# tobiTKM/SPaRC-Gym

Hardware: AMD Instinct MI355X
Metric: env-steps/sec at 65,536 envs, 7x7 grid (HBM roofline fraction in 'roofline') (higher is better)
Workload: dtype u8/u64 (integer bitboards)

## Files before the change

sparc-gym_amd/csrc/sparc_kernels.hip:

```cpp
#include <hip/hip_runtime.h>
#include <dlfcn.h>

#include <algorithm>
#include <atomic>
#include <cstdlib>
#include <cstdio>
#include <cstring>
#include <mutex>
#include <string>
#include <thread>
#include <type_traits>
#include <vector>

#include "sparc_env.hpp"
#include "sparc_trie.hpp"
#include "sparc_movew.hpp"
#include "sparc_move1.hpp"
#include "sparc_rules.hpp"
#include "sparc_snapshot.hpp"
#include "sparc_expand.hpp"
#include "sparc_devbuf.hpp"
#include "sparc_tables.hpp"
#include "sparc_gym_amd.h"

// ... 1040 lines not shown
            }
            if constexpr (!LDS_TABLE) m.tile_end();
            __syncthreads();
        }
        __syncthreads();
        __syncthreads();
        uint4 fs = fin[0], fc;
        if constexpr (IOR) {
            const int32_t* cnt = reinterpret_cast<const int32_t*>(smem + kS_Cnt) + pr * 64u + lane;
            fc = make_uint4((uint32_t)cnt[256], fs.z, 0u, 0u);
            fs.z = (uint32_t)cnt[0];
            fs.w = (uint32_t)cnt[512];
        } else {
            fc = fin[1];
        }
        const uint32_t pend = m.pending ? 1u : 0u;
        m.store(p, i, col, col_addr, fs.x, pend ? (fs.y == 0u ? 1u : 2u) : 0u, fc.y);
        if (stats) {
            const uint32_t resets = p.autoreset == 1 ? pend0 + fc.x - pend : 0u;
            int4 st = stats[i];
            st.x += (int)fs.z;
            st.y += (int)fc.x;
            st.z += (int)fs.w;
            st.w += (int)resets;
            stats[i] = st;
        }
    } else {
        __builtin_amdgcn_s_setprio(1);
        static_assert(!(C && LA), "compact records: the plain trie wave only");
        using TL = TrieLaneT<C>;
        using Rec = typename TL::Rec;
        const Rec* trie = reinterpret_cast<const Rec*>(p.tab.trie8);
        TL tl;
        tl.load(p.st.pos[i], p.st.aux[i], p.st.pid[i], trow, trie, NP);
        const uint32_t* th = reinterpret_cast<const uint32_t*>(pb + kS_FH) + lane;
        uint8_t* tr = pb + kS_Rew + lane;
        static_assert(!(LA && RAND), "the look-ahead trie wave reads the next tile's actions from HBM tiles");
        __syncthreads();
        __syncthreads();
        if constexpr (LA)
            if (K > 0) tl.prime(pb[kS_Act + lane], p.tab.trieg);
        if constexpr (!LDS_TABLE) {
            tl.slot_addr = slot_addr;
            tl.lim = kRowSlots;
        }
        for (int32_t k = 1; k <= K; ++k) {
            const uint8_t* ta = pb + kS_Act + ((k - 1) % 3) * (kTile * 64) + lane;
            if constexpr (!LDS_TABLE) tl.slot_read(kRowSlots, kRowSlotStride);
            const uint32_t a_next = LA ? pb[kS_Act + (k % 3) * (kTile * 64) + lane] : 0u;
#pragma unroll 1
            for (int g = 0; g < kTile; g += kGroup1s) {
                const uint32_t row0 = (uint32_t)((k - 1) * kTile + g) & (kRing - 1);
                uint32_t hb[kGroup1s], av[kGroup1s + 1];
#pragma unroll
                for (int j = 0; j < kGroup1s; ++j) {
                    hb[j] = th[(row0 + j) * 64];
                    av[j] = ta[(g + j) * 64];
                }
                if constexpr (LA) av[kGroup1s] = g + kGroup1s < kTile ? (uint32_t)ta[(g + kGroup1s) * 64] : a_next;
#pragma unroll
                for (int j = 0; j < kGroup1s; ++j) {
                    int code;
                    if constexpr (LA) code = tl.template step1la<!IOR>(hb[j], av[j], av[j + 1], trow, p.tab.trieg, NP);
                    else if constexpr (LDS_TABLE) code = tl.template step1<!IOR>(hb[j], av[j], trow, trie, NP);
                    else code = tl.template step1s<!IOR, kRowSlots, kRowSlotStride>(hb[j], av[j], trow, trie, NP);
                    tr[(row0 + j) * 64] = (uint8_t)code;
                }
            }
            if constexpr (!LDS_TABLE) tl.slot_tile_end(kRowSlots);
            __syncthreads();
        }
        if constexpr (IOR)
            if (K > 0) tl.finish_oneg(th[((uint32_t)(K * kTile - 1) & (kRing - 1)) * 64u] & kHwDone);
        if constexpr (IOR) {
            fin[0] = make_uint4(tl.std_S(), (uint32_t)tl.Oneg, tl.pid, 0u);
        } else {
            fin[0] = make_uint4(tl.std_S(), (uint32_t)tl.Oneg, (uint32_t)tl.acc_x, tl.acc_z);
            fin[1] = make_uint4(tl.acc_y, tl.pid, 0u, 0u);
        }
        __syncthreads();
    }
}

template <int G, int A, int RT>
struct R1Geom {
    static_assert(G * (1 + A) <= 16 && RT % A == 0, "k_rollout1r shape");
    static constexpr int kBlock = 64 * G * (1 + A);
    static constexpr uint32_t kEnvs = 64u * G;
    static constexpr size_t kRing = 0;
    static constexpr size_t kPid = kRing + 2 * RT * kEnvs * 8;
    static constexpr size_t kRew = kPid + 2 * RT * kEnvs * 4;
    static constexpr size_t kFlg = kRew + 3 * RT * kEnvs;
    static constexpr size_t kBits = kFlg + 3 * RT * kEnvs;
    static constexpr size_t kAct = kBits + 2 * RT * kEnvs * 2;
    static constexpr size_t kStk = kAct + G * RT * 64;
    static constexpr size_t kSimple = kStk + (size_t)G * 64 * 64;
    static constexpr size_t kBase = kSimple + 512;
};

template <bool TB, bool RAND, bool LDS_TABLE, int G, int A, int RT, bool INC = false, int WPE = 6>
__global__ void __launch_bounds__(64 * G * (1 + A)) __attribute__((amdgpu_waves_per_eu(WPE)))
    k_rollout1r(Params p, int32_t T, const uint8_t* __restrict__ act, uint64_t seed, uint64_t t0,
                int8_t* __restrict__ rew, uint8_t* __restrict__ flg, int4* __restrict__ stats, uint32_t tiled,
                RulesTab rt, uint16_t* __restrict__ bits) {
    using Geo = R1Geom<G, A, RT>;
    constexpr uint32_t E = Geo::kEnvs;
    extern __shared__ __attribute__((aligned(16))) uint8_t smem[];
    const uint32_t lane = threadIdx.x & 63u, wv = threadIdx.x >> 6;
    const uint32_t g = wv % (uint32_t)G;
    const size_t n = p.n;
    const uint32_t wg_base = blockIdx.x * E;
    const uint32_t col = g * 64u + lane;
    const uint32_t i = wg_base + col;
    const bool active = i < n;
    const bool full = tiled && (size_t)wg_base + E <= n;
    const int32_t K = (T + RT - 1) / RT;
    uint64_t* ring = reinterpret_cast<uint64_t*>(smem + Geo::kRing);
    uint32_t* rpid = reinterpret_cast<uint32_t*>(smem + Geo::kPid);
    uint8_t* trw = smem + Geo::kRew;
    uint8_t* tfl = smem + Geo::kFlg;
    uint16_t* tbt = reinterpret_cast<uint16_t*>(smem + Geo::kBits);
    auto at = [](uint32_t b, int32_t j, uint32_t c) { return (b * (uint32_t)RT + (uint32_t)j) * E + c; };
    auto tile_cnt = [&](int32_t k) { return T - k * RT < RT ? T - k * RT : RT; };
    PuzzleSrc<1> src{p.tab.info, p.tab.root, p.tab.open, p.tab.init, p.tab.row1};
    if constexpr (INC) {
        for (uint32_t k = threadIdx.x; k < 512u; k += Geo::kBlock) smem[Geo::kSimple + k] = (uint8_t)ring_simple(k);
    }
    if constexpr (LDS_TABLE) {
        const uint32_t P = p.tab.num_puzzles;
        uint4* lrow1 = reinterpret_cast<uint4*>(smem + Geo::kBase);
        uint64_t* linit = reinterpret_cast<uint64_t*>(lrow1 + P);
        for (uint32_t k = threadIdx.x; k < P; k += Geo::kBlock) {
            lrow1[k] = p.tab.row1[k];
            linit[k] = p.tab.init[k];
        }
        __syncthreads();
        src = PuzzleSrc<1>{p.tab.info, p.tab.root, p.tab.open, linit, lrow1};
    }

    if (wv < (uint32_t)G) {
        using Stack = typename std::conditional<TB, LdsStack<64>, RegStack>::type;
        Env<1, TB, Stack> e;
        if constexpr (TB) e.stk.col = smem + Geo::kStk + g * 4096u + lane;
        int4 acc = make_int4(0, 0, 0, 0);
        uint64_t initc = 0;
        uint32_t sbit = 0;
        if (active) {
            e.load(p, src, i);
            int c0;
            uint32_t s0;
            e.replay_outputs(c0, s0);
            acc.x -= c0;
            acc.z -= (int)s0;
            initc = src.get_init(e.pid);
            sbit = src.get_row1(e.pid).x & 0xFFu;
        }
        const uint64_t gid = p.env_offset + i;
        uint8_t* ta = smem + Geo::kAct + g * (RT * 64u);
        const uint32_t r = lane >> 2, c = (lane & 3u) * 16u;
        const bool tact = !RAND && full;
        u32x4 anext = {0u, 0u, 0u, 0u};
        if (tact && (int32_t)r < tile_cnt(0)) anext = nt_load16(act + (size_t)r * n + wg_base + g * 64u + c);
        auto store_rf = [&](int32_t kt) {
            const int32_t cnt = tile_cnt(kt);
            const uint32_t b = (uint32_t)kt % 3u;
            if (full) {
                constexpr uint32_t kPer = E / 16u;
                for (uint32_t pi = col; pi < kPer * (uint32_t)cnt; pi += E) {
                    const uint32_t row = pi / kPer, cb = (pi % kPer) * 16u;
                    const size_t o = (size_t)(kt * RT + (int32_t)row) * n + wg_base + cb;
                    if (rew) nt_store16(reinterpret_cast<uint8_t*>(rew) + o, *reinterpret_cast<const u32x4*>(trw + at(b, (int32_t)row, cb)));
                    if (flg) nt_store16(flg + o, *reinterpret_cast<const u32x4*>(tfl + at(b, (int32_t)row, cb)));
                }
            } else if (active) {
                for (int32_t j = 0; j < cnt; ++j) {
                    const size_t o = (size_t)(kt * RT + j) * n + i;
                    if (rew) rew[o] = (int8_t)trw[at(b, j, col)];
                    if (flg) flg[o] = tfl[at(b, j, col)];
                }
            }
        };
        auto store_bits = [&](int32_t kt) {
            const int32_t cnt = tile_cnt(kt);
            const uint32_t b = (uint32_t)kt & 1u;
            if (full) {
                constexpr uint32_t kPer = E / 8u;
                for (uint32_t pi = col; pi < kPer * (uint32_t)cnt; pi += E) {
                    const uint32_t row = pi / kPer, ce = (pi % kPer) * 8u;
                    const size_t o = (size_t)(kt * RT + (int32_t)row) * n + wg_base + ce;
                    nt_store16(reinterpret_cast<uint8_t*>(bits + o), *reinterpret_cast<const u32x4*>(tbt + at(b, (int32_t)row, ce)));
                }
            } else if (active) {
                for (int32_t j = 0; j < cnt; ++j) bits[(size_t)(kt * RT + j) * n + i] = tbt[at(b, j, col)];
            }
        };
        __syncthreads();
        for (int32_t k = 0; k < K; ++k) {
            const int32_t cnt = tile_cnt(k);
            const uint32_t b = (uint32_t)k & 1u;
            if (tact) {
                const u32x4 acur = anext;
                if (k + 1 < K && (int32_t)r < tile_cnt(k + 1))
                    anext = nt_load16(act + (size_t)((k + 1) * RT + (int32_t)r) * n + wg_base + g * 64u + c);
                if ((int32_t)r < cnt) *reinterpret_cast<u32x4*>(ta + r * 64u + c) = acur;
                wave_lds_fence();
            }
#pragma unroll 1
            for (int32_t j = 0; j < cnt; ++j) {
                const int32_t t = k * RT + j;
                uint32_t a = 0;
                if constexpr (RAND) a = uint_rand_action(seed, gid, t0 + (uint64_t)t);
                else if (tact) a = ta[j * 64 + (int32_t)lane];
                else if (active) a = act[(size_t)t * n + i];
                uint32_t f = 0;
                uint64_t w = 0;
                uint32_t q_after = 0;
                if (active) {
                    e.reset_next(p, src);
                    if (e.rs) {
                        initc = e.fr;
                        sbit = e.e;
                    }
                    const int code = e.phase_trie(p);
                    f = e.phase_move(p, a);
                    acc.x += code;
                    acc.z += (int)e.solved;
                    acc.y += (int)e.pending;
                    acc.w += (int)e.s_rs;
                    if (t > 0) {
                        const int32_t tp = t - 1;
                        trw[((uint32_t)(tp / RT) % 3u * (uint32_t)RT + (uint32_t)(tp % RT)) * E + col] = (uint8_t)code;
                    }
                    w = (((initc & ~e.fr) >> p.pitch) | (1ull << sbit)) | ((uint64_t)e.e << kRingShift);
                    q_after = e.pid;
                }
                ring[at(b, j, col)] = w;
                rpid[at(b, j, col)] = q_after;
                tfl[((uint32_t)k % 3u * (uint32_t)RT + (uint32_t)j) * E + col] = (uint8_t)f;
            }
            if (k >= 2) {
                store_rf(k - 2);
                store_bits(k - 2);
            }
            __syncthreads();
        }
        if (active) {
            const int code = e.phase_trie(p);
            acc.x += code;
            acc.z += (int)e.solved;
            const int32_t tp = T - 1;
            trw[((uint32_t)(tp / RT) % 3u * (uint32_t)RT + (uint32_t)(tp % RT)) * E + col] = (uint8_t)code;
        }
        if (K >= 2) {
            store_rf(K - 2);
            store_bits(K - 2);
        }
        __syncthreads();
        store_rf(K - 1);
        store_bits(K - 1);
        if (!active) return;
        e.store(p, src, i);
        if (stats) {
            int4 st = stats[i];
            st.x += acc.x;
            st.y += acc.y;
            st.z += acc.z;
            st.w += acc.w;
            stats[i] = st;
        }
        return;
    }

    __builtin_amdgcn_s_setprio(1);
    const uint32_t q = wv / (uint32_t)G - 1u;
    PuzzleRules<1> pr;
    pr.q = 0xFFFFFFFFu;
    __syncthreads();
    __syncthreads();
    if constexpr (INC) {
        constexpr int32_t BL = RT / A;
        const uint8_t* simple = smem + Geo::kSimple;
        RegionSet1 rs;
        for (int32_t k = 1; k <= K; ++k) {
            const int32_t kt = k - 1, cnt = tile_cnt(kt);
            const uint32_t b = (uint32_t)kt & 1u;
            const int32_t j0 = (int32_t)q * BL, j1 = j0 + BL < cnt ? j0 + BL : cnt;
            if (A > 1) rs.q = 0xFFFFFFFFu;
#pragma unroll 1
            for (int32_t j = j0; j < j1; ++j) {
                const uint64_t w = ring[at(b, j, col)];
                const uint32_t pid = rpid[at(b, j, col)];
                uint32_t out = 0;
                if (active) {
                    if (pr.q != pid) pr = puzzle_rules<1>(p, rt, pid);
                    const uint32_t ab = (uint32_t)(w >> kRingShift) & 63u;
                    out = rs.audit(p, rt, pr, w & ((1ull << kRingShift) - 1ull), ab == pr.tbit, simple);
                }
                tbt[at(b, j, col)] = (uint16_t)out;
            }
            __syncthreads();
        }
        return;
    }
    constexpr uint32_t kSlots = (uint32_t)(A * G) * 64u;
    const uint32_t s0 = (wv - (uint32_t)G) * 64u + lane;
    (void)q;
    for (int32_t k = 1; k <= K; ++k) {
        const int32_t kt = k - 1, cnt = tile_cnt(kt);
        const uint32_t b = (uint32_t)kt & 1u;
#pragma unroll 1
        for (uint32_t J = s0; J < (uint32_t)RT * E; J += kSlots) {
            const uint32_t ec = J / (uint32_t)RT, jj = J - ec * (uint32_t)RT;
            const int32_t j = (int32_t)jj;
            if (j >= cnt) continue;
            const uint64_t w = ring[at(b, j, ec)];
            const uint32_t pid = rpid[at(b, j, ec)];
            uint32_t out = 0;
            if (wg_base + ec < n) {
                if (pid != pr.q) pr = puzzle_rules<1>(p, rt, pid);
                BB<1> vb;
                vb.w[0] = w & ((1ull << kRingShift) - 1ull);
                const uint32_t ab = (uint32_t)(w >> kRingShift) & 63u;
                out = audit_r<1, NoMemo, true>(p, rt, pr, vb, ab == pr.tbit, nullptr, nullptr).bits;
            }
            tbt[at(b, j, ec)] = (uint16_t)out;
        }
        __syncthreads();
    }
}

constexpr size_t kW_Act = 0, kW_Rew = 2 * kTile * 64, kW_Hand = kW_Rew + kRing * 64, kW_Board = kW_Hand + 2 * kRing * 64;
__host__ __device__ constexpr size_t splitw_fin_bytes() { return 4 * 64 * 2 * sizeof(uint4); }

template <int W, bool TB, bool RAND, bool LDS_TABLE, bool IOR = false>
__global__ void __launch_bounds__(kBlock1s) k_rolloutWs(Params p, SplitGeom g, const uint4* __restrict__ mrow,
                                                        const uint32_t* __restrict__ boards, int32_t T,
                                                        const uint8_t* __restrict__ act, uint64_t seed, uint64_t t0,
                                                        int8_t* __restrict__ rew, uint8_t* __restrict__ flg,
                                                        int4* __restrict__ stats) {
    extern __shared__ __attribute__((aligned(16))) uint8_t smem[];
    const uint32_t lane = threadIdx.x & 63u, wv = threadIdx.x >> 6;
    const uint32_t NP = p.tab.num_puzzles;
    const size_t fin_off = 4 * (size_t)g.pair;
    const uint4* trow = p.tab.trow;
    if constexpr (LDS_TABLE) {
        uint4* lt = reinterpret_cast<uint4*>(smem + fin_off + splitw_fin_bytes());
        for (uint32_t k = threadIdx.x; k < NP; k += kBlock1s) lt[k] = p.tab.trow[k];
        __syncthreads();
        trow = lt;
    }
    const size_t n = p.n;
    const uint32_t wg_base = blockIdx.x * 256u;
    const int32_t K = T / kTile;

    int32_t* const cnt = reinterpret_cast<int32_t*>(smem + fin_off + 256 * sizeof(uint4));
    if (wv >= 8) {
        const uint32_t io = wv - 8u;
        const uint32_t r = lane >> 2, c = (lane & 3u) * 16u;
        IoCounters ct;
        auto load_tile = [&](int32_t k) {
            if constexpr (!RAND) {
// ... 325 lines not shown
    int dev = -1;
    DevGuard() {
        if (hipGetDevice(&dev) != hipSuccess) dev = -1;
    }
    ~DevGuard() {
        int cur = -1;
        if (dev >= 0 && hipGetDevice(&cur) == hipSuccess && cur != dev) (void)hipSetDevice(dev);
    }
    DevGuard(const DevGuard&) = delete;
    DevGuard& operator=(const DevGuard&) = delete;
};

Params make_params(const Ctx* c, const PuzzleDev& z) {
    Params p{};
    p.tab.open = z.open.get();
    p.tab.info = z.info.get();
    p.tab.root = z.root.get();
    p.tab.trie = z.trie.get();
    p.tab.init = z.init.get();
    p.tab.row1 = z.row1.get();
    p.tab.trie8 = z.trie8.get();
    p.tab.trieg = z.trieg.get();
    p.tab.trow = z.trow.get();
    p.tab.mrow = z.mrow.get();
    p.tab.num_puzzles = z.num_puzzles;
    p.st.vis = c->vis.get();
    p.st.dirs = c->dirs.get();
    p.st.pos = c->pos.get();
    p.st.aux = c->aux.get();
    p.st.step = c->step.get();
    p.st.pid = c->pid.get();
    p.n = c->n;
    p.pitch = (uint32_t)c->cfg.pitch;
    p.max_steps = c->cfg.max_steps;
    p.autoreset = c->cfg.autoreset;
    p.env_offset = (uint64_t)c->cfg.env_offset;
    p.err = c->err.get();
    const uint32_t P = p.pitch;
    p.nbr_pos = (2u * P) | ((P - 1u) << 8) | (0u << 16) | ((P + 1u) << 24);
    if (c->W == 1 && split1_pitch_ok(P)) {
        p.nbm = window_nbm(P);
        p.lmagic = legal_magic(P);
    }
    return p;
}
Params make_params(const Ctx* c) { return make_params(c, c->pz); }

inline dim3 grid_for(size_t n) { return dim3((unsigned)((n + kBlock - 1) / kBlock)); }

int allow_big_lds(Ctx* c, const void* kern) {
    static std::mutex mu;
    static std::vector<std::pair<int, const void*>> done;
    std::lock_guard<std::mutex> lock(mu);
    for (const auto& k : done)
        if (k.first == c->device && k.second == kern) return SPARC_OK;
    HIPCHK(c, hipFuncSetAttribute(kern, hipFuncAttributeMaxDynamicSharedMemorySize, (int)kMaxDynLds));
    done.emplace_back(c->device, kern);
    return SPARC_OK;
}

template <class F>
void dispatch_w_tb(int w, bool tb, F&& f) {
    using T1 = std::integral_constant<int, 1>;
    using T2 = std::integral_constant<int, 2>;
    using T4 = std::integral_constant<int, 4>;
    if (w == 1) tb ? f(T1{}, std::true_type{}) : f(T1{}, std::false_type{});
    else if (w == 2) tb ? f(T2{}, std::true_type{}) : f(T2{}, std::false_type{});
    else tb ? f(T4{}, std::true_type{}) : f(T4{}, std::false_type{});
}

int check_ctx(Ctx* c, bool need_state) {
    if (!c) return fail(nullptr, SPARC_E_INVALID, "null context");
    if (!c->loaded) return fail(c, SPARC_E_STATE, "sparc_load_puzzles has not been called");
    if (need_state && !c->has_state) return fail(c, SPARC_E_STATE, "sparc_reset has not been called");
    HIPCHK(c, hipSetDevice(c->device));
    return SPARC_OK;
}

int launch_check(Ctx* c) {
    HIPCHK(c, hipGetLastError());
    return SPARC_OK;
}

template <int G_, int A_, int RT_, bool INC_ = false, int WPE_ = 6>
struct R1Shape {
    static constexpr int G = G_, A = A_, RT = RT_, WPE = WPE_;
    static constexpr bool INC = INC_;
};

constexpr uint64_t kFitQueueCap = 1u << 16;
constexpr uint64_t kFitQueueMax = (uint64_t)1 << 28;

RulesTab rules_tab(const Ctx* c, const RuleDev& r, bool queue) {
    RulesTab rt{};
    rt.planes = r.planes.get();
    rt.inst_fc = r.inst_fc.get();
    rt.inst = r.inst.get();
    rt.shape_range = r.shape_range.get();
    rt.shape_area = r.shape_area.get();
    rt.shape_off = r.shape_off.get();
    rt.num_puzzles = c->pz.num_puzzles;
    rt.area = r.area ? 1u : 0u;
    rt.fit_cap = c->fit_cap;
    rt.reg_off = r.reg_off.get();
    rt.reg_tab = r.reg_tab.get();
    rt.fq = FitQueue{queue ? c->fq_count.get() : nullptr, c->fq_items.get(), c->fq_items.size()};
    rt.hf = c->hostfits_off ? HostFits{nullptr, 0u, 0u}
                            : HostFits{c->d_hf.get(), c->h_hf.empty() ? 0u : (uint32_t)c->h_hf.size() - 1u, c->d_hf ? c->hf_used : 0u};
    rt.rows = r.rows.get();
    return rt;
}

template <int W>
int host_fit_w(const Ctx* c, const RuleDev& r, uint32_t q, uint64_t rm) {
    const uint32_t w0 = c->pz.h_info[q].x, X = w0 & 0xFFu, Y = (w0 >> 8) & 0xFFu;
    RulesTab rt{};
    rt.inst = r.h_inst.data();
    rt.shape_range = r.h_shape_range.data();
    rt.shape_off = r.h_shape_off.data();
    const uint2 fc = r.h_inst_fc[q];
    const FitIn fin = fit_in(rt, fc.x, fc.y & ~kHostFit, X, Y);
    const uint32_t P = (uint32_t)c->cfg.pitch;
    BB<W> Rc = BB<W>::zero();
    for (uint32_t b = 0; b < fin.CX * fin.CY; ++b)
        if ((rm >> b) & 1ull) Rc.set((2 * (b / fin.CY) + 1) * P + 2 * (b % fin.CY) + 1);
    if (fc.y & kHostFit) return exact_fit<W, uint64_t, kHostFitMax, kHostFitMax, kHostFitPlanes>(fin, Rc, rm, ~0ull);
    return exact_fit<W, uint64_t>(fin, Rc, rm, ~0ull);
}
int host_fit(const Ctx* c, const RuleDev& r, uint32_t q, uint64_t rm) {
    return c->W == 1 ? host_fit_w<1>(c, r, q, rm) : c->W == 2 ? host_fit_w<2>(c, r, q, rm) : host_fit_w<4>(c, r, q, rm);
}

template <class F>
void parallel_for(size_t n, F&& fn) {
    std::atomic<size_t> next{0};
    auto work = [&]() {
        for (size_t k; (k = next.fetch_add(1)) < n;) fn(k);
    };
    const size_t nt = std::min<size_t>({n, 16, (size_t)std::max(1u, std::thread::hardware_concurrency())});
    std::vector<std::thread> pool;
    for (size_t k = 1; k < nt; ++k) pool.emplace_back(work);
    work();
    for (auto& th : pool) th.join();
}

}

extern "C" {

int sparc_abi_version(void) { return SPARC_ABI_VERSION; }

const char* sparc_last_error(const void* ctx) {
    return ctx ? static_cast<const Ctx*>(ctx)->msg.c_str() : g_err.c_str();
}

int sparc_create(int device, const sparc_config* cfg, void** ctx_out) {
    DevGuard dg;
    if (!cfg || !ctx_out) return fail(nullptr, SPARC_E_INVALID, "null argument");
    *ctx_out = nullptr;
    if (cfg->num_envs < 1) return fail(nullptr, SPARC_E_INVALID, "num_envs must be >= 1");
    if (cfg->words != 1 && cfg->words != 2 && cfg->words != 4)
        return fail(nullptr, SPARC_E_INVALID, "words must be 1, 2 or 4");
    if (cfg->pitch < 1 || cfg->pitch > 255) return fail(nullptr, SPARC_E_INVALID, "pitch must be in 1..255");
    if (cfg->traceback != 0 && cfg->traceback != 1) return fail(nullptr, SPARC_E_INVALID, "traceback must be 0/1");
    if (cfg->autoreset != SPARC_AUTORESET_NONE && cfg->autoreset != SPARC_AUTORESET_NEXT_STEP)
        return fail(nullptr, SPARC_E_INVALID, "unknown autoreset mode");
    int ndev = 0;
    if (hipGetDeviceCount(&ndev) != hipSuccess || ndev == 0)
        return fail(nullptr, SPARC_E_HIP, "no HIP device available");
    if (device < 0 || device >= ndev) return fail(nullptr, SPARC_E_INVALID, "bad device ordinal");
    Ctx* c = new Ctx();
// ... 222 lines not shown
                           (!rtr || aligned(rtr->bits));
    const bool half = false;
    if (c->W == 1 && !ot && !rtr) {
        const size_t blocks = (c->n + 255) / 256;
        const size_t per_cu = (blocks + 255) / 256;
        const size_t budget = std::min(kMaxDynLds, (size_t)160 * 1024 / (per_cu ? per_cu : 1));
        const size_t tbytes = table_lds_bytes<1>(c->pz.num_puzzles);
        if (tiled && c->n % 256 == 0 && T >= kTile && c->pz.trie8 && split1_pitch_ok((uint32_t)c->cfg.pitch)) {
            const int32_t T16 = T / kTile * kTile;
            const size_t sbytes = split_table_bytes(c->pz.num_puzzles);
            const bool lds_s = kS_Base + sbytes <= budget;
            const size_t shm_s = kS_Base + (lds_s ? sbytes : kS_SlotBytes);
            const bool compact = !lds_s && c->pz.trie4 && (c->mixed_trie == 1 || (c->mixed_trie == 0 && c->pz.mixed_pays));
            Params ps = p;
            if (compact) {
                ps.tab.trie8 = reinterpret_cast<const uint2*>(c->pz.trie4.get());
                ps.tab.trow = c->pz.trow4.get();
            }
            auto launch_s = [&](auto kern, const uint8_t* a) {
                if (shm_s > 64 * 1024 && (lds_rc = allow_big_lds(c, reinterpret_cast<const void*>(kern)))) return;
                kern<<<dim3((unsigned)blocks), kBlock1s, shm_s, c->stream>>>(ps, T16, a, seed, t0, d_rew, d_flags, st);
            };
            auto launch_s1 = [&](auto kern, const uint8_t* a) {
                if (shm_s > 64 * 1024 && (lds_rc = allow_big_lds(c, reinterpret_cast<const void*>(kern)))) return;
                kern<<<dim3((unsigned)(4 * blocks)), kBlock1s / 4, shm_s, c->stream>>>(ps, T16, a, seed, t0, d_rew, d_flags,
                                                                                     st);
            };
            auto go_s = [&](auto tb, auto ior) {
                constexpr bool TB = decltype(tb)::value, IOR = decltype(ior)::value;
                if (d_act) {
                    if (lds_s && blocks <= 64) launch_s1(k_rollout1s<TB, false, true, true, IOR, false, 1>, d_act);
                    else if (lds_s) launch_s(k_rollout1s<TB, false, true, false, IOR>, d_act);
                    else if (compact) launch_s(k_rollout1s<TB, false, false, false, IOR, true>, d_act);
                    else launch_s(k_rollout1s<TB, false, false, false, IOR>, d_act);
                } else {
                    if (lds_s) launch_s(k_rollout1s<TB, true, true, false, IOR>, nullptr);
                    else if (compact) launch_s(k_rollout1s<TB, true, false, false, IOR, true>, nullptr);
                    else launch_s(k_rollout1s<TB, true, false, false, IOR>, nullptr);
                }
            };
            const bool ior = p.autoreset == 1 && !c->io_codes_off;
            if (c->cfg.traceback) {
                if (ior) go_s(std::true_type{}, std::true_type{});
                else go_s(std::true_type{}, std::false_type{});
            } else {
                if (ior) go_s(std::false_type{}, std::true_type{});
                else go_s(std::false_type{}, std::false_type{});
            }
            if (lds_rc) return lds_rc;
            rc = launch_check(c);
            if (rc || T16 == T) return rc;
            const size_t adv = (size_t)T16 * c->n;
            if (d_act) d_act += adv;
            if (d_rew) d_rew += adv;
            if (d_flags) d_flags += adv;
            t0 += (uint64_t)T16;
            T -= T16;
        }
        const bool lds_table = kW1Base + tbytes <= budget;
        const size_t shm = kW1Base + (lds_table ? tbytes : 0);
        auto launch = [&](auto kern, const uint8_t* a) {
            if (shm > 64 * 1024 && (lds_rc = allow_big_lds(c, reinterpret_cast<const void*>(kern)))) return;
            kern<<<dim3((unsigned)blocks), kBlock1, shm, c->stream>>>(p, T, a, seed, t0, d_rew, d_flags, st, tiled);
        };
        auto go1 = [&](auto tb) {
            constexpr bool TB = decltype(tb)::value;
            if (d_act) {
                if (lds_table) launch(k_rollout1<TB, false, true>, d_act);
                else launch(k_rollout1<TB, false, false>, d_act);
            } else {
                if (lds_table) launch(k_rollout1<TB, true, true>, nullptr);
                else launch(k_rollout1<TB, true, false>, nullptr);
            }
        };
        if (c->cfg.traceback) go1(std::true_type{});
        else go1(std::false_type{});
        if (lds_rc) return lds_rc;
        return launch_check(c);
    }
    if (rtr && r1r_rollout(c)) {
        auto go_shape = [&](auto geo_c) {
            using Geo = decltype(geo_c);
            constexpr int G = Geo::G, A = Geo::A, RT = Geo::RT, WPE = Geo::WPE;
            constexpr bool INC = Geo::INC;
            using GG = R1Geom<G, A, RT>;
            const size_t blocks = (c->n + GG::kEnvs - 1) / GG::kEnvs;
            const size_t tbytes = table_lds_bytes<1>(c->pz.num_puzzles);
            const bool lds_table = GG::kBase + tbytes <= (GG::kBlock <= 768 ? (size_t)80 * 1024 : kMaxDynLds);
            const size_t shm = GG::kBase + (lds_table ? tbytes : 0);
            auto launch = [&](auto kern, const uint8_t* a) {
                if (shm > 64 * 1024 && (lds_rc = allow_big_lds(c, reinterpret_cast<const void*>(kern)))) return;
                kern<<<dim3((unsigned)blocks), GG::kBlock, shm, c->stream>>>(p, T, a, seed, t0, d_rew, d_flags, st, tiled,
                                                                            rtr->rt, rtr->bits);
            };
            auto go = [&](auto tb) {
                constexpr bool TB = decltype(tb)::value;
                if (d_act) {
                    if (lds_table) launch(k_rollout1r<TB, false, true, G, A, RT, INC, WPE>, d_act);
                    else launch(k_rollout1r<TB, false, false, G, A, RT, INC, WPE>, d_act);
                } else {
                    if (lds_table) launch(k_rollout1r<TB, true, true, G, A, RT, INC, WPE>, nullptr);
                    else launch(k_rollout1r<TB, true, false, G, A, RT, INC, WPE>, nullptr);
                }
            };
            if (c->cfg.traceback) go(std::true_type{});
            else go(std::false_type{});
        };
        switch (c->r1r_shape) {
            case 1: go_shape(R1Shape<4, 3, 12>{}); break;
            case 2: go_shape(R1Shape<2, 4, 12>{}); break;
            case 3: go_shape(R1Shape<4, 1, 4, true, 4>{}); break;
            case 4: go_shape(R1Shape<2, 3, 15, true, 4>{}); break;
            case 5: go_shape(R1Shape<2, 5, 10>{}); break;
            default: go_shape(R1Shape<2, 5, 15>{}); break;
        }
        if (lds_rc) return lds_rc;
        return launch_check(c);
    }
    if (c->W > 1 && !ot && !rtr && c->pz.split_w && tiled && c->n % 256 == 0 && T >= kTile) {
        const int32_t T16 = T / kTile * kTile;
        const SplitGeom& g = c->pz.sgeom;
        const size_t blocks = c->n / 256;
        const size_t base = 4 * (size_t)g.pair + splitw_fin_bytes();
        const bool lds_t = base + sizeof(uint4) * c->pz.num_puzzles <= kMaxDynLds;
        const size_t shm = base + (lds_t ? sizeof(uint4) * c->pz.num_puzzles : 0);
        dispatch_w_tb(c->W, c->cfg.traceback, [&](auto w, auto tb) {
            constexpr int W = decltype(w)::value;
            constexpr bool TB = decltype(tb)::value;
            if constexpr (W > 1) {
                auto launch = [&](auto kern, const uint8_t* a) {
                    if (shm > 64 * 1024 && (lds_rc = allow_big_lds(c, reinterpret_cast<const void*>(kern)))) return;
                    kern<<<dim3((unsigned)blocks), kBlock1s, shm, c->stream>>>(p, g, c->pz.mroww.get(), c->pz.boardw.get(), T16, a, seed,
                                                                              t0, d_rew, d_flags, st);
                };
                auto go = [&](auto ior) {
                    constexpr bool IOR = decltype(ior)::value;
                    if (d_act) {
                        if (lds_t) launch(k_rolloutWs<W, TB, false, true, IOR>, d_act);
                        else launch(k_rolloutWs<W, TB, false, false, IOR>, d_act);
                    } else {
                        if (lds_t) launch(k_rolloutWs<W, TB, true, true, IOR>, nullptr);
                        else launch(k_rolloutWs<W, TB, true, false, IOR>, nullptr);
                    }
                };
                if (p.autoreset == 1 && !c->io_codes_off) go(std::true_type{});
                else go(std::false_type{});
            }
        });
        if (lds_rc) return lds_rc;
        rc = launch_check(c);
        if (rc || T16 == T) return rc;
        const size_t adv = (size_t)T16 * c->n;
        if (d_act) d_act += adv;
        if (d_rew) d_rew += adv;
        if (d_flags) d_flags += adv;
        t0 += (uint64_t)T16;
        T -= T16;
    }
    if (ot && !c->obs_inline) {
        dispatch_w_tb(c->W, c->cfg.traceback, [&](auto w, auto tb) {
            constexpr int W = decltype(w)::value;
            constexpr bool TB = decltype(tb)::value;
            const size_t shm = obsw_lds_bytes<W, TB>();
            const dim3 g((unsigned)((c->n + 255) / 256));
            auto launch = [&](auto kern, const uint8_t* a) {
                if (shm > 64 * 1024 && (lds_rc = allow_big_lds(c, reinterpret_cast<const void*>(kern)))) return;
                kern<<<g, kBlockOw, shm, c->stream>>>(p, T, a, seed, t0, d_rew, d_flags, st, *ot);
            };
            if (d_act) launch(k_rollout_obsw<W, TB, false>, d_act);
            else launch(k_rollout_obsw<W, TB, true>, nullptr);
        });
        if (lds_rc) return lds_rc;
        return launch_check(c);
    }
    dispatch_w_tb(c->W, c->cfg.traceback, [&](auto w, auto tb) {
        constexpr int W = decltype(w)::value;
        constexpr bool TB = decltype(tb)::value;
        auto go = [&](auto epw_c, auto obs_c, auto rules_c) {
            constexpr int EPW = decltype(epw_c)::value;
            constexpr bool OBS = decltype(obs_c)::value;
            constexpr bool RULES = decltype(rules_c)::value;
            if constexpr (W == 1 && !OBS && !RULES) return;
            constexpr size_t kEnvsPerBlock = (size_t)kWaves * EPW / (RULES ? kAuditWaves : 1);
            const size_t blocks = (c->n + kEnvsPerBlock - 1) / kEnvsPerBlock;
            const size_t per_cu = (blocks + 255) / 256;
            const size_t budget = std::min(kMaxDynLds, (size_t)160 * 1024 / (per_cu ? per_cu : 1));
            const size_t base = tiles_lds_bytes<W, EPW>() + stack_lds_bytes<W, TB, EPW>() + (OBS ? obs_lds_bytes<W>() : 0) +
                                (RULES ? bits_lds_bytes<EPW>() : 0);
            const size_t tbytes = table_lds_bytes<W>(c->pz.num_puzzles);
            const bool lds_table = base + tbytes <= budget;
            const size_t shm = base + (lds_table ? tbytes : 0);
            const dim3 g((unsigned)blocks);
            auto launch = [&](auto kern, const uint8_t* a) {
                if (shm > 64 * 1024 && (lds_rc = allow_big_lds(c, reinterpret_cast<const void*>(kern)))) return;
                kern<<<g, kBlock, shm, c->stream>>>(p, T, a, seed, t0, d_rew, d_flags, st, tiled, ot ? *ot : no_obs,
                                                    rtr ? *rtr : no_rules);
            };
// ... 295 lines not shown
        if (cnt > c->fq_items.size()) return fail(c, SPARC_E_STATE, "exact-fit queue overflow on the re-run");
    }
    std::vector<FitTodo> todo(cnt);
    HIPCHK(c, hipMemcpy(todo.data(), c->fq_items.get(), sizeof(FitTodo) * cnt, hipMemcpyDeviceToHost));
    c->fq_last = cnt;
    for (const FitTodo& it : todo)
        if (it.pos >= a.extent || it.q >= c->pz.num_puzzles)
            return fail(c, SPARC_E_STATE, "exact-fit queue entry outside the last audit call");
    std::vector<std::pair<uint32_t, uint64_t>> keys(cnt);
    for (uint64_t k = 0; k < cnt; ++k) keys[k] = {todo[k].q, todo[k].rm};
    std::sort(keys.begin(), keys.end());
    keys.erase(std::unique(keys.begin(), keys.end()), keys.end());
    std::vector<int8_t> res(keys.size(), 0);
    parallel_for(keys.size(), [&](size_t k) { res[k] = (int8_t)host_fit(c, c->rl, keys[k].first, keys[k].second); });
    auto fits = [&](uint32_t q, uint64_t rm) {
        const auto it = std::lower_bound(keys.begin(), keys.end(), std::make_pair(q, rm));
        return res[(size_t)(it - keys.begin())] == 1;
    };
    std::sort(todo.begin(), todo.end(), [](const FitTodo& x, const FitTodo& y) { return x.pos < y.pos; });
    std::vector<RulePatch> patch;
    for (size_t k = 0; k < todo.size();) {
        RulePatch r{todo[k].pos, 0ull, SPARC_RULE_SEARCH_EXHAUSTED, 0u};
        bool ok = true;
        for (; k < todo.size() && todo[k].pos == r.pos; ++k) {
            const bool f = fits(todo[k].q, todo[k].rm);
            ok &= f;
            if (f) r.fit_or |= 1ull << (todo[k].rid & 63u);
        }
        if (!ok) r.clear |= SPARC_RULE_POLY_YLOP | SPARC_RULE_ALL;
        patch.push_back(r);
    }
    DevBuf<RulePatch> d_patch;
    HIPCHK(c, upload(d_patch, patch, c->stream));
    k_rule_patch<<<grid_for(patch.size()), kBlock, 0, c->stream>>>(d_patch.get(), (uint32_t)patch.size(), d_bits, d_fit);
    rc = launch_check(c);
    HIPCHK(c, hipMemsetAsync(c->fq_count.get(), 0, sizeof(unsigned long long), c->stream));
    if (!rc) rc = hostfits_add(c, keys, res);
    HIPCHK(c, hipStreamSynchronize(c->stream));
    return rc;
}
}

extern "C" {

int sparc_rules_device(void* ctx, uint16_t* d_bits, uint8_t* d_region, uint64_t* d_fit) {
    DevGuard dg;
    Ctx* c = static_cast<Ctx*>(ctx);
    int rc = check_ctx(c, true);
    if (rc) return rc;
    if (!c->rules) return fail(c, SPARC_E_STATE, "sparc_load_rules has not been called");
    HIPCHK(c, hipMemsetAsync(c->fq_count.get(), 0, sizeof(unsigned long long), c->stream));
    AuditCall a;
    a.kind = 1;
    a.extent = c->n;
    a.bits = d_bits;
    a.region = d_region;
    a.fit = d_fit;
    c->last_audit = a;
    return launch_rules(c, a);
}

int sparc_rules_queue_stats(void* ctx, uint64_t* out) {
    Ctx* c = static_cast<Ctx*>(ctx);
    if (!c || !out) return fail(c, SPARC_E_INVALID, "null argument");
    out[0] = c->fq_items.size();
    out[1] = c->fq_last;
    out[2] = c->fq_reruns;
    return SPARC_OK;
}

int sparc_set_variant(void* ctx, int32_t which, int32_t value) {
    Ctx* c = static_cast<Ctx*>(ctx);
    if (!c) return fail(nullptr, SPARC_E_INVALID, "null context");
    switch (which) {
        case SPARC_VARIANT_IO_CODES_OFF:
            if (value != 0 && value != 1) break;
            c->io_codes_off = value == 1;
            return SPARC_OK;
        case SPARC_VARIANT_RULE_ROLLOUT_GENERIC:
            if (value != 0 && value != 1) break;
            c->rules_generic = value == 1;
            return SPARC_OK;
        case SPARC_VARIANT_R1R_SHAPE:
            if (value < 0 || value > 5) break;
            c->r1r_shape = value;
            return SPARC_OK;
        case SPARC_VARIANT_OBS_INLINE:
            if (value != 0 && value != 1) break;
            c->obs_inline = value == 1;
            return SPARC_OK;
        case SPARC_VARIANT_MIXED_TRIE:
            if (value < 0 || value > 2) break;
            c->mixed_trie = value;
            return SPARC_OK;
        case SPARC_VARIANT_HOST_FITS:
            if (value != 0 && value != 1) break;
            c->hostfits_off = value == 1;
            return SPARC_OK;
        default:
            return fail(c, SPARC_E_INVALID, "unknown variant");
    }
    return fail(c, SPARC_E_INVALID, "bad variant value");
}

int sparc_set_rule_limits(void* ctx, uint32_t fit_cap_nodes, uint64_t table_entries) {
    DevGuard dg;
    Ctx* c = static_cast<Ctx*>(ctx);
    if (!c) return fail(nullptr, SPARC_E_INVALID, "null context");
    c->fit_cap = fit_cap_nodes ? fit_cap_nodes : kFitCap;
    c->reg_entries = table_entries ? (size_t)std::min<uint64_t>(table_entries, (uint64_t)1 << 28) : (size_t)1 << 28;
    return SPARC_OK;
}

int sparc_rules_finish(void* ctx, uint16_t* d_bits, uint64_t* d_fit) {
    DevGuard dg;
    Ctx* c = static_cast<Ctx*>(ctx);
    int rc = check_ctx(c, false);
    if (rc) return rc;
    if (!c->rules) return fail(c, SPARC_E_STATE, "sparc_load_rules has not been called");
    uint64_t cnt = 0;
    if ((rc = read_queue_count(c, cnt))) return rc;
    return finish_queue(c, cnt, d_bits, d_fit);
}

int sparc_rules_host(void* ctx, uint16_t* bits, uint8_t* region, uint64_t* fit) {
    DevGuard dg;
    Ctx* c = static_cast<Ctx*>(ctx);
    int rc = check_ctx(c, true);
    if (rc) return rc;
    const size_t n = c->n, rb = n * 64 * c->W;
    if ((rc = audit_scratch(c))) return rc;
    rc = sparc_rules_device(c, c->s_bits.get(), region ? c->s_region.get() : nullptr, fit ? c->s_fit.get() : nullptr);
    if (rc) return rc;
    HIPCHK(c, c->h_count.ensure(hipHostMallocDefault));
    HIPCHK(c, hipMemcpyAsync(c->h_count.get(), c->fq_count.get(), sizeof(uint64_t), hipMemcpyDeviceToHost, c->stream));
    if (bits) HIPCHK(c, hipMemcpyAsync(bits, c->s_bits.get(), 2 * n, hipMemcpyDeviceToHost, c->stream));
    if (region) HIPCHK(c, hipMemcpyAsync(region, c->s_region.get(), rb, hipMemcpyDeviceToHost, c->stream));
    if (fit) HIPCHK(c, hipMemcpyAsync(fit, c->s_fit.get(), 8 * n, hipMemcpyDeviceToHost, c->stream));
    HIPCHK(c, hipStreamSynchronize(c->stream));
    const uint64_t cnt = *c->h_count.get();
    if ((rc = finish_queue(c, cnt, c->s_bits.get(), fit ? c->s_fit.get() : nullptr)) || cnt == 0) return rc;
    if (bits) HIPCHK(c, hipMemcpyAsync(bits, c->s_bits.get(), 2 * n, hipMemcpyDeviceToHost, c->stream));
    if (fit) HIPCHK(c, hipMemcpyAsync(fit, c->s_fit.get(), 8 * n, hipMemcpyDeviceToHost, c->stream));
    return sparc_sync(c);
}

}

namespace {
int env_call(Ctx* c, int32_t env, int32_t op, uint32_t arg, int32_t audit, sparc_env_record* out) {
    int rc = check_ctx(c, op != 2);
    if (rc) return rc;
    if (!out) return fail(c, SPARC_E_INVALID, "null record");
    if (env < 0 || (uint32_t)env >= c->n) return fail(c, SPARC_E_INVALID, "env index out of range");
    if (op == 2 && !c->has_state && c->n != 1)
        return fail(c, SPARC_E_STATE, "first reset must cover every env (sparc_reset_*)");
    if (op == 2 && arg >= c->pz.num_puzzles) return fail(c, SPARC_E_INVALID, "puzzle index out of range");
    if (audit && !c->rules) return fail(c, SPARC_E_STATE, "sparc_load_rules has not been called");
    HIPCHK(c, c->h_rec.ensure(hipHostMallocMapped));
    const Params p = make_params(c);
    dispatch_w_tb(c->W, c->cfg.traceback, [&](auto w, auto tb) {
        k_env_op<decltype(w)::value, decltype(tb)::value><<<1, 64, 0, c->stream>>>(p, (uint32_t)env, op, arg, c->h_rec.dev());
    });
    if ((rc = launch_check(c))) return rc;
    if (op == 2) c->has_state = true;
    if (audit) {
        if ((rc = audit_scratch(c))) return rc;
// ... 477 lines not shown
```

sparc-gym_amd/csrc/sparc_layout.hpp:

```cpp
#pragma once
#include <stddef.h>
#include <stdint.h>

#if defined(__HIP__)
#define SPARC_HD __attribute__((host)) __attribute__((device))
#else
#define SPARC_HD
#endif

namespace sparc {

constexpr uint32_t kNone = 0xFFFFu;
constexpr size_t kMaxDynLds = 160 * 1024;

SPARC_HD constexpr bool split1_pitch_ok(uint32_t P) { return P >= 3u && P <= 9u; }

struct SplitGeom {
    uint32_t P2;
    uint32_t B;
    uint32_t BS;
    uint32_t M;
    uint32_t nbr_pos;
    uint32_t pair;
    uint32_t off_board, off_stack;
};
constexpr uint32_t kBoardRegs = 4;

constexpr uint32_t kRingShift = 57;

constexpr size_t kMixedTrieBytes = (size_t)4 << 20;
constexpr uint32_t kHotWalk = 8;

enum : uint32_t {
    RP_CELLS = 0, RP_LATTICE, RP_GAPS, RP_DOTS, RP_TRI, RP_TRI0, RP_TRI1, RP_TRI2, RP_STAR, RP_SQUARE,
    RP_COLORED, RP_COL1, RP_M0 = RP_COL1 + 8, RP_M1, RP_M2, RP_NOTFIRST, RP_NOTLAST, RP_INST, RP_ABI,
    RP_AREA0 = RP_ABI, RP_COUNT = RP_AREA0 + 8
};
constexpr int kAreaPlanes = 8;
constexpr int kFitYlops = 16;
constexpr int kFitShapes = 16;
constexpr int kHostFitMax = 64, kHostFitPlanes = 8;
constexpr uint32_t kHostFit = 0x80000000u;

SPARC_HD inline __attribute__((always_inline)) uint32_t hostfit_slot(uint32_t q, uint64_t rm, uint32_t mask) {
    uint64_t h = rm * 0x9E3779B97F4A7C15ull ^ ((uint64_t)q * 0xC2B2AE3D27D4EB4Full);
    h ^= h >> 29;
    return (uint32_t)h & mask;
}

template <int W>
SPARC_HD constexpr uint32_t rule_row_u64() { return 10u * W + 2u; }
constexpr uint32_t kBasePlanes[10] = {RP_CELLS, RP_LATTICE, RP_GAPS, RP_DOTS, RP_TRI, RP_TRI0, RP_TRI1, RP_TRI2,
                                      RP_NOTFIRST, RP_NOTLAST};
constexpr uint32_t kNoRegTab = 0xFFFFFFFFu;
constexpr uint32_t kRegTabCells = 12;

}
```

Before: 411.5 billion.

## Deduplicate identical audit jobs per tile and compact them into an LDS job list

Adds a DISTINCT variant of the rollout kernel where audit waves first find, for each env within a tile, the steps whose ring word and puzzle id match an earlier step. Only the first occurrence of each is kept, and those are compacted via ballot, atomicAdd and mbcnt into a shared-memory job list. Audit waves then balance work across the compacted list and copy each result to the duplicate steps. Extra __syncthreads are added so producer waves hand off mid-tile. This becomes the new default shape and costs extra LDS, barriers and equality-scan work.

```diff
diff --git a/sparc-gym_amd/csrc/sparc_kernels.hip b/sparc-gym_amd/csrc/sparc_kernels.hip
--- a/sparc-gym_amd/csrc/sparc_kernels.hip
+++ b/sparc-gym_amd/csrc/sparc_kernels.hip
@@ -1146,9 +1146,9 @@
     }
 }
 
-template <int G, int A, int RT>
+template <int G, int A, int RT, bool DISTINCT = false>
 struct R1Geom {
-    static_assert(G * (1 + A) <= 16 && RT % A == 0, "k_rollout1r shape");
+    static_assert(G * (1 + A) <= 16 && (RT % A == 0 || DISTINCT), "k_rollout1r shape");
     static constexpr int kBlock = 64 * G * (1 + A);
     static constexpr uint32_t kEnvs = 64u * G;
     static constexpr size_t kRing = 0;
@@ -1159,15 +1159,20 @@
     static constexpr size_t kAct = kBits + 2 * RT * kEnvs * 2;
     static constexpr size_t kStk = kAct + G * RT * 64;
     static constexpr size_t kSimple = kStk + (size_t)G * 64 * 64;
-    static constexpr size_t kBase = kSimple + 512;
+    static constexpr size_t kList = kSimple + 512;
+    static constexpr size_t kBase = kList + (DISTINCT ? 2 * RT * kEnvs + 16 : 0);
+    static_assert(!DISTINCT || (RT <= 16 && kEnvs <= 4096u), "a job is ec << 4 | j in 16 bits");
 };
 
-template <bool TB, bool RAND, bool LDS_TABLE, int G, int A, int RT, bool INC = false, int WPE = 6>
+template <bool TB, bool RAND, bool LDS_TABLE, int G, int A, int RT, bool INC = false, int WPE = 6, bool DISTINCT = false>
 __global__ void __launch_bounds__(64 * G * (1 + A)) __attribute__((amdgpu_waves_per_eu(WPE)))
     k_rollout1r(Params p, int32_t T, const uint8_t* __restrict__ act, uint64_t seed, uint64_t t0,
                 int8_t* __restrict__ rew, uint8_t* __restrict__ flg, int4* __restrict__ stats, uint32_t tiled,
                 RulesTab rt, uint16_t* __restrict__ bits) {
-    using Geo = R1Geom<G, A, RT>;
+    static_assert(!(INC && DISTINCT), "k_rollout1r: INC keeps regions from step to step, DISTINCT skips steps");
+    constexpr int32_t kMarkSteps = 4;
+    (void)kMarkSteps;
+    using Geo = R1Geom<G, A, RT, DISTINCT>;
     constexpr uint32_t E = Geo::kEnvs;
     extern __shared__ __attribute__((aligned(16))) uint8_t smem[];
     const uint32_t lane = threadIdx.x & 63u, wv = threadIdx.x >> 6;
@@ -1190,6 +1195,13 @@
     if constexpr (INC) {
         for (uint32_t k = threadIdx.x; k < 512u; k += Geo::kBlock) smem[Geo::kSimple + k] = (uint8_t)ring_simple(k);
     }
+    uint16_t* jlist = reinterpret_cast<uint16_t*>(smem + Geo::kList);
+    uint32_t* jcnt = reinterpret_cast<uint32_t*>(smem + Geo::kList + 2 * RT * E);
+    if constexpr (DISTINCT) {
+        if (threadIdx.x < 2u) jcnt[threadIdx.x] = 0u;
+    }
+    (void)jlist;
+    (void)jcnt;
     if constexpr (LDS_TABLE) {
         const uint32_t P = p.tab.num_puzzles;
         uint4* lrow1 = reinterpret_cast<uint4*>(smem + Geo::kBase);
@@ -1204,6 +1216,7 @@
 
     if (wv < (uint32_t)G) {
         using Stack = typename std::conditional<TB, LdsStack<64>, RegStack>::type;
+        if constexpr (DISTINCT) __builtin_amdgcn_s_setprio(1);
         Env<1, TB, Stack> e;
         if constexpr (TB) e.stk.col = smem + Geo::kStk + g * 4096u + lane;
         int4 acc = make_int4(0, 0, 0, 0);
@@ -1271,6 +1284,9 @@
             }
 #pragma unroll 1
             for (int32_t j = 0; j < cnt; ++j) {
+                if constexpr (DISTINCT) {
+                    if (j == kMarkSteps) __syncthreads();
+                }
                 const int32_t t = k * RT + j;
                 uint32_t a = 0;
                 if constexpr (RAND) a = uint_rand_action(seed, gid, t0 + (uint64_t)t);
@@ -1302,6 +1318,9 @@
                 rpid[at(b, j, col)] = q_after;
                 tfl[((uint32_t)k % 3u * (uint32_t)RT + (uint32_t)j) * E + col] = (uint8_t)f;
             }
+            if constexpr (DISTINCT) {
+                if (cnt <= kMarkSteps) __syncthreads();
+            }
             if (k >= 2) {
                 store_rf(k - 2);
                 store_bits(k - 2);
@@ -1315,6 +1334,7 @@
             const int32_t tp = T - 1;
             trw[((uint32_t)(tp / RT) % 3u * (uint32_t)RT + (uint32_t)(tp % RT)) * E + col] = (uint8_t)code;
         }
+        if constexpr (DISTINCT) __syncthreads();
         if (K >= 2) {
             store_rf(K - 2);
             store_bits(K - 2);
@@ -1335,12 +1355,73 @@
         return;
     }
 
-    __builtin_amdgcn_s_setprio(1);
+    if constexpr (!DISTINCT) __builtin_amdgcn_s_setprio(1);
     const uint32_t q = wv / (uint32_t)G - 1u;
     PuzzleRules<1> pr;
     pr.q = 0xFFFFFFFFu;
     __syncthreads();
+    if constexpr (DISTINCT) __syncthreads();
     __syncthreads();
+    if constexpr (DISTINCT) {
+        constexpr uint32_t kSlots = (uint32_t)(A * G) * 64u;
+        constexpr uint32_t kJobs = (uint32_t)RT * E;
+        constexpr uint32_t kRounds = (kJobs + kSlots - 1u) / kSlots;
+        const uint32_t aw = wv - (uint32_t)G;
+        const uint32_t s0 = aw * 64u + lane;
+        for (int32_t k = 1; k <= K; ++k) {
+            const int32_t kt = k - 1, cnt = tile_cnt(kt);
+            const uint32_t b = (uint32_t)kt & 1u;
+            const uint64_t* rw = ring + at(b, 0, 0);
+            const uint32_t* rq = rpid + at(b, 0, 0);
+            uint32_t* const cw = jcnt + ((uint32_t)k & 1u);
+            uint64_t own[kRounds];
+            uint32_t total = 0;
+#pragma unroll
+            for (uint32_t r = 0; r < kRounds; ++r) {
+                const uint32_t J = (aw * kRounds + r) * 64u + lane;
+                const uint32_t ec = J / (uint32_t)RT, j = J - ec * (uint32_t)RT;
+                bool mine = false;
+                if (J < kJobs && (int32_t)j < cnt) {
+                    if (wg_base + ec < n) mine = tile_rep(tile_equal_mask<RT>(rw + ec, rq + ec, E, j), j) == j;
+                    else tbt[at(b, (int32_t)j, ec)] = 0;
+                }
+                own[r] = __ballot(mine);
+                total += (uint32_t)__popcll(own[r]);
+            }
+            uint32_t base = 0;
+            if (lane == 0u && total) base = atomicAdd(cw, total);
+            base = (uint32_t)__builtin_amdgcn_readfirstlane((int)base);
+#pragma unroll
+            for (uint32_t r = 0; r < kRounds; ++r) {
+                const uint32_t J = (aw * kRounds + r) * 64u + lane;
+                const uint32_t ec = J / (uint32_t)RT, j = J - ec * (uint32_t)RT;
+                const uint32_t rank = __builtin_amdgcn_mbcnt_hi((uint32_t)(own[r] >> 32),
+                                                                __builtin_amdgcn_mbcnt_lo((uint32_t)own[r], 0u));
+                if (((own[r] >> lane) & 1ull) && base + rank < kJobs) jlist[base + rank] = (uint16_t)(ec << 4 | j);
+                base += (uint32_t)__popcll(own[r]);
+            }
+            __syncthreads();
+            const uint32_t listed = *cw < kJobs ? *cw : kJobs;
+            if (threadIdx.x == (uint32_t)G * 64u) jcnt[((uint32_t)k + 1u) & 1u] = 0u;
+#pragma unroll 1
+            for (uint32_t s = s0; s < listed; s += kSlots) {
+                const uint32_t e = jlist[s];
+                const uint32_t ec = e >> 4, j = e & 15u;
+                const uint64_t w = rw[j * E + ec];
+                const uint32_t pid = rq[j * E + ec];
+                if (pid != pr.q) pr = puzzle_rules<1>(p, rt, pid);
+                BB<1> vb;
+                vb.w[0] = w & ((1ull << kRingShift) - 1ull);
+                const uint32_t ab = (uint32_t)(w >> kRingShift) & 63u;
+                const uint32_t out = audit_r<1, NoMemo, true>(p, rt, pr, vb, ab == pr.tbit, nullptr, nullptr).bits;
+                tbt[at(b, (int32_t)j, ec)] = (uint16_t)out;
+                for (uint32_t f = tile_followers(tile_equal_mask<RT>(rw + ec, rq + ec, E, j), j, (uint32_t)cnt); f; f &= f - 1u)
+                    tbt[at(b, __builtin_ctz(f), ec)] = (uint16_t)out;
+            }
+            __syncthreads();
+        }
+        return;
+    }
     if constexpr (INC) {
         constexpr int32_t BL = RT / A;
         const uint8_t* simple = smem + Geo::kSimple;
@@ -1832,11 +1913,12 @@
     return SPARC_OK;
 }
 
-template <int G_, int A_, int RT_, bool INC_ = false, int WPE_ = 6>
+template <int G_, int A_, int RT_, bool INC_ = false, int WPE_ = 6, bool DISTINCT_ = false>
 struct R1Shape {
     static constexpr int G = G_, A = A_, RT = RT_, WPE = WPE_;
-    static constexpr bool INC = INC_;
+    static constexpr bool INC = INC_, DISTINCT = DISTINCT_;
 };
+constexpr int kR1rDefault = 9;
 
 constexpr uint64_t kFitQueueCap = 1u << 16;
 constexpr uint64_t kFitQueueMax = (uint64_t)1 << 28;
@@ -2225,8 +2307,8 @@
         auto go_shape = [&](auto geo_c) {
             using Geo = decltype(geo_c);
             constexpr int G = Geo::G, A = Geo::A, RT = Geo::RT, WPE = Geo::WPE;
-            constexpr bool INC = Geo::INC;
-            using GG = R1Geom<G, A, RT>;
+            constexpr bool INC = Geo::INC, DISTINCT = Geo::DISTINCT;
+            using GG = R1Geom<G, A, RT, DISTINCT>;
             const size_t blocks = (c->n + GG::kEnvs - 1) / GG::kEnvs;
             const size_t tbytes = table_lds_bytes<1>(c->pz.num_puzzles);
             const bool lds_table = GG::kBase + tbytes <= (GG::kBlock <= 768 ? (size_t)80 * 1024 : kMaxDynLds);
@@ -2239,23 +2321,26 @@
             auto go = [&](auto tb) {
                 constexpr bool TB = decltype(tb)::value;
                 if (d_act) {
-                    if (lds_table) launch(k_rollout1r<TB, false, true, G, A, RT, INC, WPE>, d_act);
-                    else launch(k_rollout1r<TB, false, false, G, A, RT, INC, WPE>, d_act);
+                    if (lds_table) launch(k_rollout1r<TB, false, true, G, A, RT, INC, WPE, DISTINCT>, d_act);
+                    else launch(k_rollout1r<TB, false, false, G, A, RT, INC, WPE, DISTINCT>, d_act);
                 } else {
-                    if (lds_table) launch(k_rollout1r<TB, true, true, G, A, RT, INC, WPE>, nullptr);
-                    else launch(k_rollout1r<TB, true, false, G, A, RT, INC, WPE>, nullptr);
+                    if (lds_table) launch(k_rollout1r<TB, true, true, G, A, RT, INC, WPE, DISTINCT>, nullptr);
+                    else launch(k_rollout1r<TB, true, false, G, A, RT, INC, WPE, DISTINCT>, nullptr);
                 }
             };
             if (c->cfg.traceback) go(std::true_type{});
             else go(std::false_type{});
         };
-        switch (c->r1r_shape) {
+        switch (c->r1r_shape ? c->r1r_shape : kR1rDefault) {
             case 1: go_shape(R1Shape<4, 3, 12>{}); break;
             case 2: go_shape(R1Shape<2, 4, 12>{}); break;
             case 3: go_shape(R1Shape<4, 1, 4, true, 4>{}); break;
             case 4: go_shape(R1Shape<2, 3, 15, true, 4>{}); break;
             case 5: go_shape(R1Shape<2, 5, 10>{}); break;
-            default: go_shape(R1Shape<2, 5, 15>{}); break;
+            case 6: go_shape(R1Shape<2, 5, 15>{}); break;
+            case 7: go_shape(R1Shape<2, 5, 13, false, 6, true>{}); break;
+            case 8: go_shape(R1Shape<2, 5, 14, false, 6, true>{}); break;
+            case 9: go_shape(R1Shape<2, 5, 15, false, 6, true>{}); break;
         }
         if (lds_rc) return lds_rc;
         return launch_check(c);
@@ -2717,7 +2802,7 @@
             c->rules_generic = value == 1;
             return SPARC_OK;
         case SPARC_VARIANT_R1R_SHAPE:
-            if (value < 0 || value > 5) break;
+            if (value < 0 || value > 9) break;
             c->r1r_shape = value;
             return SPARC_OK;
         case SPARC_VARIANT_OBS_INLINE:
diff --git a/sparc-gym_amd/csrc/sparc_layout.hpp b/sparc-gym_amd/csrc/sparc_layout.hpp
--- a/sparc-gym_amd/csrc/sparc_layout.hpp
+++ b/sparc-gym_amd/csrc/sparc_layout.hpp
@@ -28,6 +28,26 @@
 
 constexpr uint32_t kRingShift = 57;
 
+template <int RT>
+SPARC_HD inline __attribute__((always_inline)) uint32_t tile_equal_mask(const uint64_t* w, const uint32_t* q,
+                                                                         uint32_t stride, uint32_t j) {
+    static_assert(RT >= 1 && RT <= 16, "a tile's step fits the job list's 4 bits");
+    const uint64_t wj = w[j * stride];
+    const uint32_t qj = q[j * stride];
+    uint32_t m = 0;
+#pragma unroll
+    for (uint32_t jp = 0; jp < (uint32_t)RT; ++jp)
+        m |= (uint32_t)((w[jp * stride] == wj) & (q[jp * stride] == qj)) << jp;
+    return m & ~(1u << j);
+}
+SPARC_HD inline uint32_t tile_rep(uint32_t equal_mask, uint32_t j) {
+    const uint32_t lower = equal_mask & ((1u << j) - 1u);
+    return lower ? (uint32_t)__builtin_ctz(lower) : j;
+}
+SPARC_HD inline uint32_t tile_followers(uint32_t equal_mask, uint32_t j, uint32_t cnt) {
+    return equal_mask & ~((2u << j) - 1u) & ((1u << cnt) - 1u);
+}
+
 constexpr size_t kMixedTrieBytes = (size_t)4 << 20;
 constexpr uint32_t kHotWalk = 8;
 
```

Result: no change. 410.2 billion (-0.3%).
